# lambdaclass/ethrex

Hardware: NVIDIA H100
Metric: bn254_g1_msm_points_per_sec (higher is better)
Workload: dtype u32x8 Montgomery (254-bit modular integer)

## Files before the change

### ethrex_b200/csrc/msm.cu

```cuda
#include "common.cuh"
#include "tma.cuh"
#include <cstdlib>

namespace b200zk {

static constexpr int kMaxWindows = 64;
static constexpr uint32_t kMaxPipelineChunks = 64;
static constexpr int kChunk = 16;
static constexpr int kG2MinBlocks = 1;

struct MsmPlan {
  uint32_t c, W, B;
  uint32_t chunk, T;
  uint32_t merged;
  uint32_t Wr;
  uint32_t table_stride;
  uint32_t adaptive;
};

uint32_t precompute_window(size_t n) {
  uint32_t lg = 0;
  while (((size_t)1 << lg) < n) ++lg;
  if (lg >= 20) return 20;
  if (lg <= 6) return 6;
// ... 85 lines not shown

static constexpr uint32_t kHistTile = 256;
__global__ void __launch_bounds__(kHistTile) msm_hist(const void* scalars, size_t n, uint32_t flags, MsmPlan pl, uint32_t* hist, uint32_t* digits) {
  __shared__ __align__(128) uint4 tile[2][kHistTile * 2];
  __shared__ uint64_t bar[2];
  const size_t tiles = (n + kHistTile - 1) / kHistTile;
  if (threadIdx.x == 0) { tma::barrier_init(&bar[0], 1); tma::barrier_init(&bar[1], 1); tma::barrier_init_fence(); }
  __syncthreads();
  auto issue = [&](size_t tl, uint32_t buf) {
    size_t first = tl * kHistTile;
    uint32_t bytes = (uint32_t)((n - first < kHistTile ? n - first : kHistTile) * 32);
    tma::barrier_expect(&bar[buf], bytes);
    tma::bulk_load(tile[buf], reinterpret_cast<const uint8_t*>(scalars) + first * 32, bytes, &bar[buf]);
  };
  if (threadIdx.x == 0 && blockIdx.x < tiles) issue(blockIdx.x, 0);
  uint32_t it = 0;
  for (size_t tl = blockIdx.x; tl < tiles; tl += gridDim.x, ++it) {
    const uint32_t buf = it & 1;
    if (threadIdx.x == 0 && tl + gridDim.x < tiles) issue(tl + gridDim.x, buf ^ 1);
    tma::barrier_wait(&bar[buf], (it >> 1) & 1);
    const size_t i = tl * kHistTile + threadIdx.x;
    const bool live = i < n;
    uint32_t s[8] = {0, 0, 0, 0, 0, 0, 0, 0};
    if (live) decode_scalar(tile[buf][2 * threadIdx.x], tile[buf][2 * threadIdx.x + 1], flags, s);
    uint32_t carry = 0;
    for (uint32_t w = 0; w < pl.W; ++w) {
      uint32_t coef = window_bits(s, w, pl.c) + carry;
      carry = 0;
      uint32_t neg = 0, mag = coef;
      if (w + 1 < pl.W && coef >= pl.B) { carry = 1; neg = 0x80000000u; mag = (1u << pl.c) - coef; }
      uint32_t code = mag ? ((mag - 1) | neg) : kNoDigit;
      if (live) digits[(size_t)w * n + i] = code;
      uint32_t rank, gm;
      uint32_t cnt = warp_group(mag - 1, live && mag != 0, &rank, &gm, pl.adaptive != 0);
      if (live && mag && rank == 0) atomicAdd(&hist[(pl.merged ? 0 : (size_t)w * pl.B) + (mag - 1)], cnt);
    }
    __syncthreads();
  }
}

static constexpr int kScatterIlp = 4;
__global__ void __launch_bounds__(256) msm_scatter(const uint32_t* __restrict__ digits, size_t n, MsmPlan pl, uint32_t* cursor, uint32_t* idx) {
  const size_t total = (size_t)pl.W * n;
  const size_t stride = (size_t)gridDim.x * blockDim.x;
  const size_t total_pad = (total + 31) & ~(size_t)31;
  for (size_t t0 = blockIdx.x * (size_t)blockDim.x + threadIdx.x; t0 < total_pad; t0 += stride * kScatterIlp) {
    uint32_t code[kScatterIlp], g[kScatterIlp], rank[kScatterIlp], mask[kScatterIlp], base[kScatterIlp];
    size_t w[kScatterIlp];
    bool live[kScatterIlp], active[kScatterIlp];
#pragma unroll
    for (int u = 0; u < kScatterIlp; ++u) {
      const size_t t = t0 + u * stride;
      live[u] = t < total_pad;
      code[u] = (live[u] && t < total) ? __ldg(digits + t) : kNoDigit;
      active[u] = code[u] != kNoDigit;
      w[u] = live[u] ? t / n : 0;
      g[u] = (pl.merged ? 0u : (uint32_t)(w[u] * pl.B)) + (code[u] & 0x7fffffffu);
    }
#pragma unroll
    for (int u = 0; u < kScatterIlp; ++u) {
      base[u] = 0; rank[u] = 0; mask[u] = 0;
      if (live[u]) {
        uint32_t cnt = warp_group(g[u], active[u], &rank[u], &mask[u], pl.adaptive != 0);
        if (active[u] && rank[u] == 0) base[u] = atomicAdd(&cursor[g[u]], cnt);
      }
    }
#pragma unroll
    for (int u = 0; u < kScatterIlp; ++u) {
      if (live[u]) {
        uint32_t bs = __shfl_sync(mask[u], base[u], __ffs(mask[u]) - 1);
        const size_t t = t0 + u * stride;
        if (active[u]) idx[bs + rank[u]] = (uint32_t)((t - w[u] * n) + (pl.merged ? w[u] * pl.table_stride : 0)) | (code[u] & 0x80000000u);
      }
    }
  }
}

static constexpr uint32_t kSortTile = 1024;
static constexpr uint32_t kSortMaxW = 16;
static constexpr uint32_t kSortMaxBins = 1024;
static constexpr uint32_t kSortMaxFine = 2048;
static constexpr uint32_t kSortCountSub = 4;
static constexpr int kFineIlp = 8;

struct SortPlan {
  uint32_t fb;
  uint32_t C;
  uint32_t NC;
  uint32_t range;
  uint32_t G;
};
static bool make_sort_plan(size_t n, const MsmPlan& pl, int sm_count, SortPlan* sp) {
  const size_t G = (size_t)pl.Wr * pl.B;
  uint32_t kb = 0;
  while (((size_t)1 << kb) < G) ++kb;
  if (pl.W > kSortMaxW || kb < 12 || n < ((size_t)1 << 16)) return false;
  uint32_t cb = kb > 19 ? 10 : 9;
  if (kb - cb > 11) return false;
  sp->fb = kb - cb;
  sp->C = (uint32_t)((G + ((size_t)1 << sp->fb) - 1) >> sp->fb);
  sp->G = (uint32_t)G;
  uint32_t nc = (uint32_t)sm_count;
  size_t tiles = (n + kSortTile - 1) / kSortTile;
  if (nc > tiles) nc = (uint32_t)tiles;
  size_t per = ((tiles + nc - 1) / nc) * kSortTile;
  sp->NC = (uint32_t)((n + per - 1) / per);
  sp->range = (uint32_t)per;
  return true;
}

B2_D void recode_scalar(const uint32_t s[8], const MsmPlan& pl, uint32_t (&code)[kSortMaxW]) {
  uint32_t carry = 0;
#pragma unroll
  for (uint32_t w = 0; w < kSortMaxW; ++w) {
    code[w] = kNoDigit;
    if (w < pl.W) {
      uint32_t coef = window_bits(s, w, pl.c) + carry;
      carry = 0;
      uint32_t neg = 0, mag = coef;
      if (w + 1 < pl.W && coef >= pl.B) { carry = 1; neg = 0x80000000u; mag = (1u << pl.c) - coef; }
      code[w] = mag ? ((mag - 1) | neg) : kNoDigit;
    }
  }
}

__global__ void __launch_bounds__(kHistTile) msm_sort_count(const void* scalars, size_t n, uint32_t flags, MsmPlan pl, SortPlan sp, uint32_t* cnt) {
  __shared__ __align__(128) uint4 tile[2][kHistTile * 2];
  __shared__ uint64_t bar[2];
  __shared__ uint32_t sh[kSortMaxBins];
  const uint32_t r = blockIdx.x / kSortCountSub, sub = blockIdx.x % kSortCountSub;
  for (uint32_t b = threadIdx.x; b < sp.C; b += kHistTile) sh[b] = 0;
  const size_t lo = (size_t)r * sp.range, hi = lo + sp.range < n ? lo + sp.range : n;
  const size_t tiles_all = lo < hi ? (hi - lo + kHistTile - 1) / kHistTile : 0;
  const size_t per = (tiles_all + kSortCountSub - 1) / kSortCountSub;
  const size_t t0 = sub * per, t1 = t0 + per < tiles_all ? t0 + per : tiles_all;
  if (threadIdx.x == 0) { tma::barrier_init(&bar[0], 1); tma::barrier_init(&bar[1], 1); tma::barrier_init_fence(); }
  __syncthreads();
  auto issue = [&](size_t tl, uint32_t buf) {
    size_t first = lo + tl * kHistTile;
    uint32_t bytes = (uint32_t)((hi - first < kHistTile ? hi - first : kHistTile) * 32);
    tma::barrier_expect(&bar[buf], bytes);
    tma::bulk_load(tile[buf], reinterpret_cast<const uint8_t*>(scalars) + first * 32, bytes, &bar[buf]);
  };
  if (threadIdx.x == 0 && t0 < t1) issue(t0, 0);
  uint32_t it = 0;
  for (size_t tl = t0; tl < t1; ++tl, ++it) {
    const uint32_t buf = it & 1;
    if (threadIdx.x == 0 && tl + 1 < t1) issue(tl + 1, buf ^ 1);
    tma::barrier_wait(&bar[buf], (it >> 1) & 1);
    const size_t i = lo + tl * kHistTile + threadIdx.x;
    if (i < hi) {
      uint32_t s[8], code[kSortMaxW];
      decode_scalar(tile[buf][2 * threadIdx.x], tile[buf][2 * threadIdx.x + 1], flags, s);
      recode_scalar(s, pl, code);
#pragma unroll
      for (uint32_t w = 0; w < kSortMaxW; ++w)
        if (code[w] != kNoDigit) {
          const uint32_t g = (pl.merged ? 0u : w * pl.B) + (code[w] & 0x7fffffffu);
          atomicAdd(&sh[g >> sp.fb], 1u);
        }
    }
    __syncthreads();
  }
  __syncthreads();
  for (uint32_t b = threadIdx.x; b < sp.C; b += kHistTile) if (sh[b]) atomicAdd(&cnt[(size_t)b * sp.NC + r], sh[b]);
}

struct SortCoarseSmem {
  uint2 ent[kSortTile * kSortMaxW];
  uint32_t dst[kSortTile * kSortMaxW];
  uint32_t run_base[kSortMaxBins], tile_cnt[kSortMaxBins], tile_start[kSortMaxBins];
  uint32_t warp_tot[kSortTile / 32];
  uint32_t total;
};
__global__ void __launch_bounds__(kSortTile, 1) msm_sort_coarse(const void* __restrict__ scalars, size_t n, uint32_t flags, MsmPlan pl, SortPlan sp, const uint32_t* __restrict__ base,
                                                               uint2* __restrict__ ent1) {
  extern __shared__ __align__(16) uint8_t smem_raw[];
  SortCoarseSmem& sm = *reinterpret_cast<SortCoarseSmem*>(smem_raw);
  const uint32_t r = blockIdx.x, tid = threadIdx.x;
  const size_t lo = (size_t)r * sp.range, hi = lo + sp.range < n ? lo + sp.range : n;
  const uint32_t fmask = (1u << sp.fb) - 1u;
  for (uint32_t b = tid; b < sp.C; b += kSortTile) { sm.run_base[b] = __ldg(base + (size_t)b * sp.NC + r); sm.tile_cnt[b] = 0; }
  __syncthreads();
  const uint4* sc = reinterpret_cast<const uint4*>(scalars);
  for (size_t t0 = lo; t0 < hi; t0 += kSortTile) {
    const size_t i = t0 + tid;
    uint32_t code[kSortMaxW], rank[kSortMaxW];
    const bool live = i < hi;
#pragma unroll
    for (uint32_t w = 0; w < kSortMaxW; ++w) { code[w] = kNoDigit; rank[w] = 0; }
    if (live) {
      uint32_t s[8];
      decode_scalar(__ldg(sc + 2 * i), __ldg(sc + 2 * i + 1), flags, s);
      recode_scalar(s, pl, code);
#pragma unroll
      for (uint32_t w = 0; w < kSortMaxW; ++w)
        if (code[w] != kNoDigit) {
          const uint32_t g = (pl.merged ? 0u : w * pl.B) + (code[w] & 0x7fffffffu);
          rank[w] = atomicAdd(&sm.tile_cnt[g >> sp.fb], 1u);
        }
    }
    __syncthreads();
    {
      const uint32_t v = tid < sp.C ? sm.tile_cnt[tid] : 0;
      uint32_t incl = v;
#pragma unroll
      for (int o = 1; o < 32; o <<= 1) { uint32_t t = __shfl_up_sync(0xffffffffu, incl, o); if ((tid & 31) >= (unsigned)o) incl += t; }
      if ((tid & 31) == 31) sm.warp_tot[tid >> 5] = incl;
      __syncthreads();
      uint32_t wb = 0;
      for (uint32_t k = 0; k < (tid >> 5); ++k) wb += sm.warp_tot[k];
      if (tid < sp.C) sm.tile_start[tid] = wb + incl - v;
      if (tid == kSortTile - 1) sm.total = wb + incl;
    }
    __syncthreads();
    if (live) {
#pragma unroll
      for (uint32_t w = 0; w < kSortMaxW; ++w)
        if (code[w] != kNoDigit) {
          const uint32_t g = (pl.merged ? 0u : w * pl.B) + (code[w] & 0x7fffffffu);
          const uint32_t b = g >> sp.fb, pos = sm.tile_start[b] + rank[w];
          sm.ent[pos] = make_uint2((uint32_t)(i + (pl.merged ? (size_t)w * pl.table_stride : 0)) | (code[w] & 0x80000000u), g & fmask);
          sm.dst[pos] = sm.run_base[b] + rank[w];
        }
    }
    __syncthreads();
    const uint32_t total = sm.total;
    for (uint32_t t = tid; t < total; t += kSortTile) ent1[sm.dst[t]] = sm.ent[t];
    __syncthreads();
    if (tid < sp.C) { sm.run_base[tid] += sm.tile_cnt[tid]; sm.tile_cnt[tid] = 0; }
    __syncthreads();
  }
}

static constexpr uint32_t kFineTile = 8192;
static constexpr uint32_t kFineSeg = 4 * kFineTile;
struct SortFineSmem {
  uint32_t val[kFineTile], dst[kFineTile];
  uint32_t cur[kSortMaxFine], tcnt[kSortMaxFine], tstart[kSortMaxFine];
  uint32_t warp_tot[32];
  uint32_t total;
};
B2_D void scan_fine_keys(const uint32_t* in, uint32_t* out, uint32_t F, uint32_t* warp_tot, uint32_t* total) {
  const uint32_t tid = threadIdx.x, k0 = 2 * tid, k1 = 2 * tid + 1;
  const uint32_t v0 = k0 < F ? in[k0] : 0, v1 = k1 < F ? in[k1] : 0;
  uint32_t incl = v0 + v1;
#pragma unroll
  for (int o = 1; o < 32; o <<= 1) { uint32_t t = __shfl_up_sync(0xffffffffu, incl, o); if ((tid & 31) >= (unsigned)o) incl += t; }
  if ((tid & 31) == 31) warp_tot[tid >> 5] = incl;
  __syncthreads();
  uint32_t wb = 0;
  for (uint32_t k = 0; k < (tid >> 5); ++k) wb += warp_tot[k];
  const uint32_t ex = wb + incl - v0 - v1;
  if (k0 < F) out[k0] = ex;
  if (k1 < F) out[k1] = ex + v0;
  if (tid == 1023) *total = wb + incl;
  __syncthreads();
}
__global__ void __launch_bounds__(1024) msm_sort_items(const uint32_t* __restrict__ base, SortPlan sp, uint32_t* __restrict__ item_start) {
  __shared__ uint32_t wt[32];
  const uint32_t tid = threadIdx.x;
  uint32_t v = 0;
  if (tid < sp.C) { const uint32_t sz = __ldg(base + (size_t)(tid + 1) * sp.NC) - __ldg(base + (size_t)tid * sp.NC); v = (sz + kFineSeg - 1) / kFineSeg; }
  uint32_t incl = v;
#pragma unroll
  for (int o = 1; o < 32; o <<= 1) { uint32_t t = __shfl_up_sync(0xffffffffu, incl, o); if ((tid & 31) >= (unsigned)o) incl += t; }
  if ((tid & 31) == 31) wt[tid >> 5] = incl;
  __syncthreads();
  uint32_t wb = 0;
  for (uint32_t k = 0; k < (tid >> 5); ++k) wb += wt[k];
  if (tid < sp.C) item_start[tid] = wb + incl - v;
  if (tid == sp.C - 1) item_start[sp.C] = wb + incl;
}
B2_D uint32_t item_bin(const uint32_t* __restrict__ item_start, uint32_t C, uint32_t i) {
  uint32_t lo = 0, hi = C;
  while (hi - lo > 1) { uint32_t mid = (lo + hi) >> 1; if (__ldg(item_start + mid) <= i) lo = mid; else hi = mid; }
  return lo;
}
__global__ void __launch_bounds__(1024, 2) msm_sort_fine_count(const uint2* __restrict__ ent1, SortPlan sp, const uint32_t* __restrict__ base, const uint32_t* __restrict__ item_start,
                                                               uint32_t* __restrict__ cnt2) {
  __shared__ uint32_t fh[kSortMaxFine];
  const uint32_t i = blockIdx.x, tid = threadIdx.x, F = 1u << sp.fb;
  if (i >= __ldg(item_start + sp.C)) return;
  const uint32_t b = item_bin(item_start, sp.C, i);
  const uint32_t bs = __ldg(base + (size_t)b * sp.NC), be = __ldg(base + (size_t)(b + 1) * sp.NC);
  const uint32_t s0 = bs + (i - __ldg(item_start + b)) * kFineSeg, s1 = (be - s0 > kFineSeg) ? s0 + kFineSeg : be;
  for (uint32_t k = tid; k < F; k += 1024) fh[k] = 0;
  __syncthreads();
  for (uint32_t e0 = s0 + tid; e0 < s1; e0 += 1024 * kFineIlp) {
    uint32_t kk[kFineIlp];
#pragma unroll
    for (int u = 0; u < kFineIlp; ++u) { const uint32_t e = e0 + u * 1024; kk[u] = e < s1 ? __ldg(&ent1[e].y) : 0xffffffffu; }
#pragma unroll
    for (int u = 0; u < kFineIlp; ++u) if (kk[u] != 0xffffffffu) atomicAdd(&fh[kk[u]], 1u);
  }
  __syncthreads();
  for (uint32_t k = tid; k < F; k += 1024) cnt2[(size_t)i * F + k] = fh[k];
}
__global__ void __launch_bounds__(256) msm_sort_fine_prefix(SortPlan sp, const uint32_t* __restrict__ item_start, uint32_t* __restrict__ cnt2, uint32_t* __restrict__ hist) {
  const uint32_t F = 1u << sp.fb;
  const size_t t = blockIdx.x * (size_t)blockDim.x + threadIdx.x;
  if (t >= (size_t)sp.C * F) return;
  const uint32_t b = (uint32_t)(t >> sp.fb), k = (uint32_t)t & (F - 1);
  const uint32_t i0 = __ldg(item_start + b), i1 = __ldg(item_start + b + 1);
  uint32_t run = 0;
  for (uint32_t i = i0; i < i1; ++i) {
    const size_t at = (size_t)i * F + k;
    const uint32_t c = cnt2[at];
    cnt2[at] = run;
    run += c;
  }
  if (t < sp.G) hist[t] = run;
}
__global__ void __launch_bounds__(1024, 1) msm_sort_fine_place(const uint2* __restrict__ ent1, SortPlan sp, const uint32_t* __restrict__ base, const uint32_t* __restrict__ item_start,
                                                               const uint32_t* __restrict__ cnt2, const uint32_t* __restrict__ offsets, uint32_t* __restrict__ idx) {
  extern __shared__ __align__(16) uint8_t smem_raw[];
  SortFineSmem& sm = *reinterpret_cast<SortFineSmem*>(smem_raw);
  const uint32_t i = blockIdx.x, tid = threadIdx.x, F = 1u << sp.fb;
  if (i >= __ldg(item_start + sp.C)) return;
  const uint32_t b = item_bin(item_start, sp.C, i);
  const uint32_t bs = __ldg(base + (size_t)b * sp.NC), be = __ldg(base + (size_t)(b + 1) * sp.NC);
  const uint32_t s0 = bs + (i - __ldg(item_start + b)) * kFineSeg, s1 = (be - s0 > kFineSeg) ? s0 + kFineSeg : be;
  for (uint32_t k = tid; k < F; k += 1024) {
    const size_t g = (size_t)b * F + k;
    sm.cur[k] = (g < sp.G ? __ldg(offsets + g) : 0u) + __ldg(cnt2 + (size_t)i * F + k);
    sm.tcnt[k] = 0;
  }
  __syncthreads();
  for (uint32_t t0 = s0; t0 < s1; t0 += kFineTile) {
    uint2 ev[kFineTile / 1024];
    uint32_t rank[kFineTile / 1024];
#pragma unroll
    for (int u = 0; u < (int)(kFineTile / 1024); ++u) {
      const uint32_t e = t0 + u * 1024 + tid;
      ev[u] = e < s1 ? __ldg(ent1 + e) : make_uint2(0u, 0xffffffffu);
    }
#pragma unroll
    for (int u = 0; u < (int)(kFineTile / 1024); ++u) rank[u] = ev[u].y != 0xffffffffu ? atomicAdd(&sm.tcnt[ev[u].y], 1u) : 0u;
    __syncthreads();
    scan_fine_keys(sm.tcnt, sm.tstart, F, sm.warp_tot, &sm.total);
#pragma unroll
    for (int u = 0; u < (int)(kFineTile / 1024); ++u)
      if (ev[u].y != 0xffffffffu) {
        const uint32_t pos = sm.tstart[ev[u].y] + rank[u];
        sm.val[pos] = ev[u].x;
        sm.dst[pos] = sm.cur[ev[u].y] + rank[u];
      }
    __syncthreads();
    const uint32_t total = sm.total;
    for (uint32_t t = tid; t < total; t += 1024) idx[sm.dst[t]] = sm.val[t];
    __syncthreads();
    for (uint32_t k = tid; k < F; k += 1024) { sm.cur[k] += sm.tcnt[k]; sm.tcnt[k] = 0; }
    __syncthreads();
  }
}

static constexpr int kScanThreads = 256, kScanItems = 8, kScanTile = kScanThreads * kScanItems;

B2_D uint32_t scan_value(const uint32_t* in, const uint32_t* aux, size_t i, uint32_t seg, uint32_t shift) {
  uint32_t v = in[i];
  if (!seg) return (v + (1u << shift) - 1u) >> shift;
  return (v != 0 && (aux[i] % seg) != 0) ? 1u : 0u;
}

__global__ void __launch_bounds__(kScanThreads) scan_tile_sums(const uint32_t* in, const uint32_t* aux, size_t G, uint32_t seg, uint32_t shift, uint32_t* tile_sums) {
  __shared__ uint32_t red[kScanThreads / 32];
  size_t base = (size_t)blockIdx.x * kScanTile + (size_t)threadIdx.x * kScanItems;
  uint32_t s = 0;
#pragma unroll
  for (int k = 0; k < kScanItems; ++k) if (base + k < G) s += scan_value(in, aux, base + k, seg, shift);
#pragma unroll
  for (int o = 16; o; o >>= 1) s += __shfl_xor_sync(0xffffffffu, s, o);
  if ((threadIdx.x & 31) == 0) red[threadIdx.x >> 5] = s;
  __syncthreads();
  if (threadIdx.x == 0) {
    uint32_t t = 0;
    for (int k = 0; k < kScanThreads / 32; ++k) t += red[k];
    tile_sums[blockIdx.x] = t;
  }
}
__global__ void __launch_bounds__(1024) scan_tile_offsets(uint32_t* tile_sums, size_t tiles) {
  __shared__ uint32_t buf[1024];
  __shared__ uint32_t carry;
  if (threadIdx.x == 0) carry = 0;
  __syncthreads();
  for (size_t base = 0; base < tiles; base += 1024) {
    size_t i = base + threadIdx.x;
    uint32_t v = i < tiles ? tile_sums[i] : 0;
    buf[threadIdx.x] = v;
    __syncthreads();
    for (int o = 1; o < 1024; o <<= 1) {
      uint32_t t = threadIdx.x >= (unsigned)o ? buf[threadIdx.x - o] : 0;
      __syncthreads();
      buf[threadIdx.x] += t;
      __syncthreads();
    }
    uint32_t incl = buf[threadIdx.x], c0 = carry;
    __syncthreads();
    if (i < tiles) tile_sums[i] = c0 + incl - v;
    if (threadIdx.x == 1023) carry = c0 + incl;
    __syncthreads();
  }
}
__global__ void __launch_bounds__(kScanThreads) scan_apply(const uint32_t* in, const uint32_t* aux, size_t G, uint32_t seg, uint32_t shift, const uint32_t* tile_offsets, uint32_t* offsets, uint32_t* cursor) {
  __shared__ uint32_t warp_tot[kScanThreads / 32];
  size_t base = (size_t)blockIdx.x * kScanTile + (size_t)threadIdx.x * kScanItems;
  uint32_t v[kScanItems], s = 0;
#pragma unroll
  for (int k = 0; k < kScanItems; ++k) { v[k] = base + k < G ? scan_value(in, aux, base + k, seg, shift) : 0; s += v[k]; }
  uint32_t incl = s;
#pragma unroll
  for (int o = 1; o < 32; o <<= 1) { uint32_t t = __shfl_up_sync(0xffffffffu, incl, o); if ((threadIdx.x & 31) >= (unsigned)o) incl += t; }
  if ((threadIdx.x & 31) == 31) warp_tot[threadIdx.x >> 5] = incl;
  __syncthreads();
  uint32_t wbase = 0;
  for (unsigned k = 0; k < (threadIdx.x >> 5); ++k) wbase += warp_tot[k];
  uint32_t run = tile_offsets[blockIdx.x] + wbase + incl - s;
#pragma unroll
  for (int k = 0; k < kScanItems; ++k) {
    if (base + k < G) { offsets[base + k] = seg ? run + (aux[base + k] + seg - 1) / seg : run; if (cursor) cursor[base + k] = run; }
    run += v[k];
  }
  if (blockIdx.x == gridDim.x - 1 && threadIdx.x == kScanThreads - 1) offsets[G] = seg ? run + (aux[G] + seg - 1) / seg : run;
}

static constexpr uint32_t kSegLenMax = 256;
static constexpr uint32_t kTreeRadix = 64;
static constexpr uint32_t kDirectRuns = 4;

static uint32_t pick_slice_len(size_t M, size_t resident) {
  if (M == 0) return kSegLenMax;
  size_t per_thread = (M + resident - 1) / resident;
  size_t waves = (per_thread + kSegLenMax - 1) / kSegLenMax;
  size_t len = (M + resident * waves - 1) / (resident * waves);
  if (len < 16) len = 16;
  if (len > kSegLenMax) len = kSegLenMax;
  return (uint32_t)len;
// ... 480 lines not shown
  for (size_t k = 0; k < count; ++k) { XYZZ<F> p = load_xyzz<F>(partials, k); xyzz_add(acc, p); }
  Affine<F> a = xyzz_to_affine(acc);
  encode_point(out, a, native);
  *reinterpret_cast<uint32_t*>(out + 2 * FieldBytes<F>::value) = a.is_inf() ? 1u : 0u;
}

__global__ void groth16_assemble(const uint8_t* __restrict__ partials, size_t count, uint8_t* __restrict__ out) {
  if (threadIdx.x) return;
  const uint32_t which = blockIdx.x;
  uint32_t* inf = reinterpret_cast<uint32_t*>(out + 320);
  if (which == 1) {
    XYZZ<Fq2> acc = XYZZ<Fq2>::identity();
    for (size_t k = 0; k < count; ++k) { XYZZ<Fq2> p = load_xyzz<Fq2>(partials + k * 768 + 256, 0); xyzz_add(acc, p); }
    Affine<Fq2> a = xyzz_to_affine(acc);
    encode_point(out + 64, a, false);
    inf[1] = a.is_inf() ? 1u : 0u;
    return;
  }
  XYZZ<Fq> acc = XYZZ<Fq>::identity();
  const size_t off = which == 0 ? 0 : (which == 3 ? 128 : 512);
  for (size_t k = 0; k < count; ++k) {
    XYZZ<Fq> p = load_xyzz<Fq>(partials + k * 768 + off, 0);
    xyzz_add(acc, p);
    if (which == 2) { XYZZ<Fq> h = load_xyzz<Fq>(partials + k * 768 + 640, 0); xyzz_add(acc, h); }
  }
  Affine<Fq> a = xyzz_to_affine(acc);
  encode_point(out + (which == 0 ? 0 : (which == 2 ? 192 : 256)), a, false);
  inf[which == 0 ? 0 : (which == 2 ? 2 : 3)] = a.is_inf() ? 1u : 0u;
}
int groth16_assemble_dev(b200zk_ctx* ctx, const void* d_partials, size_t count, cudaStream_t st, void* d_out) {
  B2_LAUNCH(ctx, groth16_assemble, 4, 32, 0, st, (const uint8_t*)d_partials, count, (uint8_t*)d_out);
  return B200ZK_OK;
}

static inline void phase_mark(b200zk_ctx* ctx, int k, cudaStream_t st) {
  if (ctx->profiling) cudaEventRecord(ctx->ev[k], st);
}

static int g2_pair_knob() {
  static int k = -1;
  if (k < 0) { const char* e = getenv("B200ZK_G2_PAIR"); k = (e && (*e == '0' || *e == '3' || *e == '4')) ? (*e - '0') : 3; }
  return k;
}
template <class F> static size_t resident_slices(const b200zk_ctx* ctx) {
  if (IsFq2<F>::value) { const int k = g2_pair_knob(); return (size_t)ctx->sm_count * (k ? 64u * (unsigned)k : 256u); }
  return (size_t)ctx->sm_count * (sizeof(F) > 32 ? 256u : 512u);
}
template <class F>
static int launch_accumulate(b200zk_ctx* ctx, cudaStream_t st, const void* pts, const uint32_t* idx, const uint32_t* offsets, const uint32_t* run_off, uint32_t G, uint32_t L,
                             size_t slices, void* partials, uint32_t* run_bucket) {
  const unsigned agrid = (unsigned)((slices + 127) / 128);
  if constexpr (IsFq2<F>::value) {
    const int k = g2_pair_knob();
    const unsigned pgrid = (unsigned)((2 * slices + 127) / 128);
    if (k == 3) B2_LAUNCH(ctx, msm_accumulate_g2_pair<3>, pgrid, 128, 0, st, pts, idx, offsets, run_off, G, L, partials, run_bucket);
    else if (k == 4) B2_LAUNCH(ctx, msm_accumulate_g2_pair<4>, pgrid, 128, 0, st, pts, idx, offsets, run_off, G, L, partials, run_bucket);
    else B2_LAUNCH(ctx, (msm_accumulate<F, false, 1>), agrid, 128, 0, st, pts, idx, offsets, run_off, G, L, partials, run_bucket);
  } else {
    B2_LAUNCH(ctx, (msm_accumulate<F, false>), agrid, 128, 0, st, pts, idx, offsets, run_off, G, L, partials, run_bucket);
  }
  return B200ZK_OK;
}

static int legacy_sort_knob() {
  static int knob = -1;
  if (knob < 0) { const char* e = getenv("B200ZK_SORT"); knob = (e && !strcmp(e, "legacy")) ? 1 : 0; }
  return knob;
}
static double chunk_ratio_knob(double dflt) {
  const char* e = getenv("B200ZK_CHUNK_RATIO");
  double r = (e && *e) ? atof(e) : dflt;
  return (r >= 1.0 && r <= 64.0) ? r : dflt;
}
static size_t sort_ctab_bytes(int sm_count) { return (2 * ((size_t)kSortMaxBins * (size_t)sm_count + 1) + kSortMaxBins + 1) * 4; }
static size_t sort_cnt2_bytes(size_t M_max) { return (M_max / kFineSeg + kSortMaxBins + 1) * (size_t)kSortMaxFine * 4; }
static int run_two_level_sort(b200zk_ctx* ctx, const void* d_scalars, size_t n, uint32_t flags, const MsmPlan& pl, const SortPlan& sp, uint32_t* hist, uint32_t* offsets,
                              uint32_t* tsum, uint2* ent1, uint32_t* ctab, uint32_t* cnt2, uint32_t* idx, cudaStream_t st, bool mark) {
  const size_t Gc = (size_t)sp.C * sp.NC, tilesC = (Gc + kScanTile - 1) / kScanTile;
  const size_t G = sp.G, tilesG = (G + kScanTile - 1) / kScanTile;
  uint32_t *cnt = ctab, *base = ctab + Gc + 1, *item_start = base + Gc + 1;
  if (!ctx->attr_sort) {
    B2_CUDA(ctx, cudaFuncSetAttribute(msm_sort_coarse, cudaFuncAttributeMaxDynamicSharedMemorySize, (int)sizeof(SortCoarseSmem)));
    B2_CUDA(ctx, cudaFuncSetAttribute(msm_sort_fine_place, cudaFuncAttributeMaxDynamicSharedMemorySize, (int)sizeof(SortFineSmem)));
    ctx->attr_sort = true;
  }
  B2_CUDA(ctx, cudaMemsetAsync(cnt, 0, (Gc + 1) * 4, st));
  B2_LAUNCH(ctx, msm_sort_count, sp.NC * kSortCountSub, kHistTile, 0, st, d_scalars, n, flags, pl, sp, cnt);
  if (mark) phase_mark(ctx, 1, st);
  B2_LAUNCH(ctx, scan_tile_sums, (unsigned)tilesC, kScanThreads, 0, st, (const uint32_t*)cnt, (const uint32_t*)nullptr, Gc, 0u, 0u, tsum);
  B2_LAUNCH(ctx, scan_tile_offsets, 1, 1024, 0, st, tsum, tilesC);
  B2_LAUNCH(ctx, scan_apply, (unsigned)tilesC, kScanThreads, 0, st, (const uint32_t*)cnt, (const uint32_t*)nullptr, Gc, 0u, 0u, (const uint32_t*)tsum, base, (uint32_t*)nullptr);
  if (mark) phase_mark(ctx, 2, st);
  B2_LAUNCH(ctx, msm_sort_coarse, sp.NC, kSortTile, sizeof(SortCoarseSmem), st, d_scalars, n, flags, pl, sp, (const uint32_t*)base, ent1);
  const unsigned max_items = (unsigned)((n * (size_t)pl.W) / kFineSeg + sp.C + 1);
  const uint32_t F = 1u << sp.fb;
  B2_LAUNCH(ctx, msm_sort_items, 1, 1024, 0, st, (const uint32_t*)base, sp, item_start);
  B2_LAUNCH(ctx, msm_sort_fine_count, max_items, 1024, 0, st, (const uint2*)ent1, sp, (const uint32_t*)base, (const uint32_t*)item_start, cnt2);
  B2_LAUNCH(ctx, msm_sort_fine_prefix, (unsigned)(((size_t)sp.C * F + 255) / 256), 256, 0, st, sp, (const uint32_t*)item_start, cnt2, hist);
  B2_LAUNCH(ctx, scan_tile_sums, (unsigned)tilesG, kScanThreads, 0, st, (const uint32_t*)hist, (const uint32_t*)nullptr, G, 0u, 0u, tsum);
  B2_LAUNCH(ctx, scan_tile_offsets, 1, 1024, 0, st, tsum, tilesG);
  B2_LAUNCH(ctx, scan_apply, (unsigned)tilesG, kScanThreads, 0, st, (const uint32_t*)hist, (const uint32_t*)nullptr, G, 0u, 0u, (const uint32_t*)tsum, offsets, (uint32_t*)nullptr);
  B2_LAUNCH(ctx, msm_sort_fine_place, max_items, 1024, sizeof(SortFineSmem), st, (const uint2*)ent1, sp, (const uint32_t*)base, (const uint32_t*)item_start, (const uint32_t*)cnt2,
            (const uint32_t*)offsets, idx);
  return B200ZK_OK;
}

template <class F>
static int msm_run_pipelined(b200zk_ctx* ctx, const void* d_points, const void* d_scalars, const void* h_scalars, size_t n, uint32_t flags,
                             cudaStream_t st, void* d_partial, const MsmPlan& pl, uint32_t K) {
  const size_t G = (size_t)pl.Wr * pl.B;
  const size_t tiles = (G + kScanTile - 1) / kScanTile;
  const size_t xy = 4 * FieldBytes<F>::value, pt = 2 * FieldBytes<F>::value;
  size_t bnd[kMaxPipelineChunks + 1];
  uint32_t chunks = 0;
  {
    const double r = h_scalars ? chunk_ratio_knob(IsFq2<F>::value ? 12.0 : 4.0) : 1.0;
    double tot = 0, w = 1;
    for (uint32_t k = 0; k < K; ++k) { tot += w; w *= r; }
    double cum = 0; w = 1;
    bnd[0] = 0;
    for (uint32_t k = 0; k < K; ++k) {
      cum += w; w *= r;
      size_t hi = (k == K - 1) ? n : std::min(n, (((size_t)((double)n * (cum / tot))) + 1023) & ~(size_t)1023);
      if (hi > bnd[chunks]) bnd[++chunks] = hi;
    }
  }
  size_t chunk = 0;
  for (uint32_t k = 0; k < chunks; ++k) chunk = std::max(chunk, bnd[k + 1] - bnd[k]);
  const size_t Mk_max = chunk * pl.W;
  const size_t resident = resident_slices<F>(ctx);
  uint32_t Lk[kMaxPipelineChunks];
  size_t S_max = 0;
  for (uint32_t k = 0; k < chunks; ++k) {
    const size_t Mk = (bnd[k + 1] - bnd[k]) * pl.W;
    Lk[k] = pick_slice_len(Mk, resident);
    S_max = std::max(S_max, Mk / Lk[k] + 1 + G);
  }
  SortPlan sp0;
  const bool two_level = !legacy_sort_knob() && make_sort_plan(chunk, pl, ctx->sm_count, &sp0);
  const size_t Gc = (size_t)kSortMaxBins * (size_t)ctx->sm_count;
  for (int sl = 0; sl < 2; ++sl) {
    SortSlot& s = ctx->slot[sl];
    B2_TRY(ensure(ctx, s.hist, G * 4)); B2_TRY(ensure(ctx, s.offsets, (G + 1) * 4)); B2_TRY(ensure(ctx, s.cursor, G * 4));
    B2_TRY(ensure(ctx, s.run_off, (G + 1) * 4));
    B2_TRY(ensure(ctx, s.tsum, std::max(tiles, (Gc + kScanTile - 1) / kScanTile) * 4));
    B2_TRY(ensure(ctx, s.digits, Mk_max * 4)); B2_TRY(ensure(ctx, s.idx, Mk_max * 4));
    if (two_level) { B2_TRY(ensure(ctx, s.key, Mk_max * 8)); B2_TRY(ensure(ctx, s.ctab, sort_ctab_bytes(ctx->sm_count))); B2_TRY(ensure(ctx, s.cnt2, sort_cnt2_bytes(Mk_max))); }
  }
  B2_TRY(ensure(ctx, ctx->ws_buckets, S_max * xy));
  B2_TRY(ensure(ctx, ctx->ws_segbucket, S_max * 4));
  B2_TRY(ensure(ctx, ctx->ws_totals, G * xy));
  B2_TRY(ensure(ctx, ctx->ws_chunkS, (size_t)pl.Wr * pl.T * xy));
  B2_TRY(ensure(ctx, ctx->ws_chunkV, (size_t)pl.Wr * pl.T * xy));
  if (h_scalars) B2_TRY(ensure(ctx, ctx->ws_scalars, n * 32 + 32));
  const uint8_t* dsc = (const uint8_t*)(h_scalars ? ctx->ws_scalars.p : d_scalars);
  cudaStream_t cs = ctx->stream_sort;
  if (h_scalars) {
    B2_CUDA(ctx, cudaEventRecord(ctx->ev_in, st));
    B2_CUDA(ctx, cudaStreamWaitEvent(cs, ctx->ev_in, 0));
    if (chunks > kMaxPipelineChunks) return fail(ctx, B200ZK_ERR_INVALID_ARG, "msm: too many pipeline chunks");
    for (uint32_t k = 0; k < chunks; ++k) {
      const size_t lo = bnd[k], nk = bnd[k + 1] - lo;
      B2_CUDA(ctx, cudaMemcpyAsync((void*)(dsc + lo * 32), (const uint8_t*)h_scalars + lo * 32, nk * 32, cudaMemcpyHostToDevice, cs));
      B2_CUDA(ctx, cudaEventRecord(ctx->ev_up[k], cs));
    }
  }
  auto sort_chunk = [&](uint32_t k) -> int {
    const size_t lo = bnd[k], nk = bnd[k + 1] - lo;
    const uint32_t L = Lk[k];
    SortSlot& s = ctx->slot[k & 1];
    uint32_t *hist = (uint32_t*)s.hist.p, *offsets = (uint32_t*)s.offsets.p, *cursor = (uint32_t*)s.cursor.p, *run_off = (uint32_t*)s.run_off.p,
             *tsum = (uint32_t*)s.tsum.p, *digits = (uint32_t*)s.digits.p, *idx = (uint32_t*)s.idx.p;
    if (h_scalars) B2_CUDA(ctx, cudaStreamWaitEvent(st, ctx->ev_up[k], 0));
    SortPlan sp;
    const bool tl = two_level && make_sort_plan(nk, pl, ctx->sm_count, &sp);
    if (tl) {
      B2_TRY(run_two_level_sort(ctx, (const void*)(dsc + lo * 32), nk, flags, pl, sp, hist, offsets, tsum, (uint2*)s.key.p, (uint32_t*)s.ctab.p, (uint32_t*)s.cnt2.p, idx, st, false));
    } else {
      B2_CUDA(ctx, cudaMemsetAsync(hist, 0, G * 4, st));
      const unsigned sgrid = (unsigned)std::min<size_t>((nk + 255) / 256, (size_t)ctx->sm_count * 8);
      B2_LAUNCH(ctx, msm_hist, sgrid, 256, 0, st, (const void*)(dsc + lo * 32), nk, flags, pl, hist, digits);
      B2_LAUNCH(ctx, scan_tile_sums, (unsigned)tiles, kScanThreads, 0, st, hist, (const uint32_t*)nullptr, G, 0u, 0u, tsum);
      B2_LAUNCH(ctx, scan_tile_offsets, 1, 1024, 0, st, tsum, tiles);
      B2_LAUNCH(ctx, scan_apply, (unsigned)tiles, kScanThreads, 0, st, hist, (const uint32_t*)nullptr, G, 0u, 0u, tsum, offsets, cursor);
      const unsigned wgrid = (unsigned)std::min<size_t>((nk * (size_t)pl.W + 255) / 256, (size_t)ctx->sm_count * 32);
      B2_LAUNCH(ctx, msm_scatter, wgrid, 256, 0, st, (const uint32_t*)digits, nk, pl, cursor, idx);
// ... 242 lines not shown
```

Baseline: 350.3 million.

## Restructure MSM two-level sort with TMA-staged scalars and single-pass fine placement

After: 362.2 million, median of 6. +3.4%, better.

```diff
diff --git a/ethrex_b200/csrc/msm.cu b/ethrex_b200/csrc/msm.cu
--- a/ethrex_b200/csrc/msm.cu
+++ b/ethrex_b200/csrc/msm.cu
@@ -191,6 +191,7 @@
 static constexpr uint32_t kSortMaxFine = 2048;
 static constexpr uint32_t kSortCountSub = 4;
 static constexpr int kFineIlp = 8;
+static constexpr uint16_t kNoFine = 0xffffu;
 
 struct SortPlan {
   uint32_t fb;
@@ -219,16 +220,27 @@
 }
 
 B2_D void recode_scalar(const uint32_t s[8], const MsmPlan& pl, uint32_t (&code)[kSortMaxW]) {
-  uint32_t carry = 0;
+  uint32_t t[9];
+#pragma unroll
+  for (int k = 0; k < 8; ++k) t[k] = s[k];
+  t[8] = 0;
+  const uint32_t mask = (1u << pl.c) - 1u;
+  uint32_t carry = 0, off = 0;
 #pragma unroll
   for (uint32_t w = 0; w < kSortMaxW; ++w) {
     code[w] = kNoDigit;
     if (w < pl.W) {
-      uint32_t coef = window_bits(s, w, pl.c) + carry;
+      uint32_t coef = (__funnelshift_r(t[0], t[1], off) & mask) + carry;
       carry = 0;
       uint32_t neg = 0, mag = coef;
       if (w + 1 < pl.W && coef >= pl.B) { carry = 1; neg = 0x80000000u; mag = (1u << pl.c) - coef; }
       code[w] = mag ? ((mag - 1) | neg) : kNoDigit;
+      off += pl.c;
+      if (off >= 32) {
+        off -= 32;
+#pragma unroll
+        for (int k = 0; k < 8; ++k) t[k] = t[k + 1];
+      }
     }
   }
 }
@@ -275,24 +287,55 @@
   for (uint32_t b = threadIdx.x; b < sp.C; b += kHistTile) if (sh[b]) atomicAdd(&cnt[(size_t)b * sp.NC + r], sh[b]);
 }
 
+template <uint32_t kThreads, uint32_t kMax>
+B2_D void scan_block(const uint32_t* in, uint32_t* out, uint32_t count, uint32_t* warp_tot, uint32_t* total) {
+  constexpr uint32_t kPer = kMax / kThreads;
+  const uint32_t tid = threadIdx.x;
+  uint32_t v[kPer], sum = 0;
+#pragma unroll
+  for (uint32_t j = 0; j < kPer; ++j) { const uint32_t k = tid * kPer + j; v[j] = k < count ? in[k] : 0; sum += v[j]; }
+  uint32_t incl = sum;
+#pragma unroll
+  for (int o = 1; o < 32; o <<= 1) { uint32_t t = __shfl_up_sync(0xffffffffu, incl, o); if ((tid & 31) >= (unsigned)o) incl += t; }
+  if ((tid & 31) == 31) warp_tot[tid >> 5] = incl;
+  __syncthreads();
+  uint32_t ex = incl - sum;
+  for (uint32_t k = 0; k < (tid >> 5); ++k) ex += warp_tot[k];
+  if (tid == kThreads - 1) *total = ex + sum;
+#pragma unroll
+  for (uint32_t j = 0; j < kPer; ++j) { const uint32_t k = tid * kPer + j; if (k < count) out[k] = ex; ex += v[j]; }
+  __syncthreads();
+}
+
 struct SortCoarseSmem {
+  uint4 sc[2][kSortTile * 2];
   uint2 ent[kSortTile * kSortMaxW];
-  uint32_t dst[kSortTile * kSortMaxW];
   uint32_t run_base[kSortMaxBins], tile_cnt[kSortMaxBins], tile_start[kSortMaxBins];
+  uint64_t bar[2];
   uint32_t warp_tot[kSortTile / 32];
   uint32_t total;
 };
 __global__ void __launch_bounds__(kSortTile, 1) msm_sort_coarse(const void* __restrict__ scalars, size_t n, uint32_t flags, MsmPlan pl, SortPlan sp, const uint32_t* __restrict__ base,
                                                                uint2* __restrict__ ent1) {
-  extern __shared__ __align__(16) uint8_t smem_raw[];
+  extern __shared__ __align__(128) uint8_t smem_raw[];
   SortCoarseSmem& sm = *reinterpret_cast<SortCoarseSmem*>(smem_raw);
   const uint32_t r = blockIdx.x, tid = threadIdx.x;
   const size_t lo = (size_t)r * sp.range, hi = lo + sp.range < n ? lo + sp.range : n;
   const uint32_t fmask = (1u << sp.fb) - 1u;
   for (uint32_t b = tid; b < sp.C; b += kSortTile) { sm.run_base[b] = __ldg(base + (size_t)b * sp.NC + r); sm.tile_cnt[b] = 0; }
-  __syncthreads();
-  const uint4* sc = reinterpret_cast<const uint4*>(scalars);
-  for (size_t t0 = lo; t0 < hi; t0 += kSortTile) {
+  if (tid == 0) { tma::barrier_init(&sm.bar[0], 1); tma::barrier_init(&sm.bar[1], 1); tma::barrier_init_fence(); }
+  __syncthreads();
+  auto issue = [&](size_t first, uint32_t buf) {
+    const uint32_t bytes = (uint32_t)((hi - first < kSortTile ? hi - first : kSortTile) * 32);
+    tma::barrier_expect(&sm.bar[buf], bytes);
+    tma::bulk_load(sm.sc[buf], reinterpret_cast<const uint8_t*>(scalars) + first * 32, bytes, &sm.bar[buf]);
+  };
+  if (tid == 0 && lo < hi) issue(lo, 0);
+  uint32_t it = 0;
+  for (size_t t0 = lo; t0 < hi; t0 += kSortTile, ++it) {
+    const uint32_t buf = it & 1;
+    if (tid == 0 && t0 + kSortTile < hi) issue(t0 + kSortTile, buf ^ 1);
+    tma::barrier_wait(&sm.bar[buf], (it >> 1) & 1);
     const size_t i = t0 + tid;
     uint32_t code[kSortMaxW], rank[kSortMaxW];
     const bool live = i < hi;
@@ -300,7 +343,7 @@
     for (uint32_t w = 0; w < kSortMaxW; ++w) { code[w] = kNoDigit; rank[w] = 0; }
     if (live) {
       uint32_t s[8];
-      decode_scalar(__ldg(sc + 2 * i), __ldg(sc + 2 * i + 1), flags, s);
+      decode_scalar(sm.sc[buf][2 * tid], sm.sc[buf][2 * tid + 1], flags, s);
       recode_scalar(s, pl, code);
 #pragma unroll
       for (uint32_t w = 0; w < kSortMaxW; ++w)
@@ -310,62 +353,40 @@
         }
     }
     __syncthreads();
-    {
-      const uint32_t v = tid < sp.C ? sm.tile_cnt[tid] : 0;
-      uint32_t incl = v;
-#pragma unroll
-      for (int o = 1; o < 32; o <<= 1) { uint32_t t = __shfl_up_sync(0xffffffffu, incl, o); if ((tid & 31) >= (unsigned)o) incl += t; }
-      if ((tid & 31) == 31) sm.warp_tot[tid >> 5] = incl;
-      __syncthreads();
-      uint32_t wb = 0;
-      for (uint32_t k = 0; k < (tid >> 5); ++k) wb += sm.warp_tot[k];
-      if (tid < sp.C) sm.tile_start[tid] = wb + incl - v;
-      if (tid == kSortTile - 1) sm.total = wb + incl;
-    }
-    __syncthreads();
+    scan_block<kSortTile, kSortMaxBins>(sm.tile_cnt, sm.tile_start, sp.C, sm.warp_tot, &sm.total);
     if (live) {
 #pragma unroll
       for (uint32_t w = 0; w < kSortMaxW; ++w)
         if (code[w] != kNoDigit) {
           const uint32_t g = (pl.merged ? 0u : w * pl.B) + (code[w] & 0x7fffffffu);
-          const uint32_t b = g >> sp.fb, pos = sm.tile_start[b] + rank[w];
-          sm.ent[pos] = make_uint2((uint32_t)(i + (pl.merged ? (size_t)w * pl.table_stride : 0)) | (code[w] & 0x80000000u), g & fmask);
-          sm.dst[pos] = sm.run_base[b] + rank[w];
+          const uint32_t pos = sm.tile_start[g >> sp.fb] + rank[w];
+          sm.ent[pos] = make_uint2((uint32_t)(i + (pl.merged ? (size_t)w * pl.table_stride : 0)) | (code[w] & 0x80000000u), g);
         }
     }
     __syncthreads();
     const uint32_t total = sm.total;
-    for (uint32_t t = tid; t < total; t += kSortTile) ent1[sm.dst[t]] = sm.ent[t];
+    for (uint32_t t = tid; t < total; t += kSortTile) {
+      const uint2 e = sm.ent[t];
+      const uint32_t b = e.y >> sp.fb;
+      ent1[sm.run_base[b] + (t - sm.tile_start[b])] = make_uint2(e.x, e.y & fmask);
+    }
     __syncthreads();
-    if (tid < sp.C) { sm.run_base[tid] += sm.tile_cnt[tid]; sm.tile_cnt[tid] = 0; }
+    for (uint32_t b = tid; b < sp.C; b += kSortTile) { sm.run_base[b] += sm.tile_cnt[b]; sm.tile_cnt[b] = 0; }
     __syncthreads();
   }
 }
 
-static constexpr uint32_t kFineTile = 8192;
-static constexpr uint32_t kFineSeg = 4 * kFineTile;
+static constexpr uint32_t kFineSeg = 32768;
+static constexpr uint32_t kFineThreads = 1024;
 struct SortFineSmem {
-  uint32_t val[kFineTile], dst[kFineTile];
-  uint32_t cur[kSortMaxFine], tcnt[kSortMaxFine], tstart[kSortMaxFine];
-  uint32_t warp_tot[32];
+  uint32_t val[kFineSeg];
+  uint16_t key[kFineSeg];
+  uint32_t cnt[kSortMaxFine];
+  uint32_t slot[kSortMaxFine];
+  uint32_t shift[kSortMaxFine];
+  uint32_t warp_tot[kFineThreads / 32];
   uint32_t total;
 };
-B2_D void scan_fine_keys(const uint32_t* in, uint32_t* out, uint32_t F, uint32_t* warp_tot, uint32_t* total) {
-  const uint32_t tid = threadIdx.x, k0 = 2 * tid, k1 = 2 * tid + 1;
-  const uint32_t v0 = k0 < F ? in[k0] : 0, v1 = k1 < F ? in[k1] : 0;
-  uint32_t incl = v0 + v1;
-#pragma unroll
-  for (int o = 1; o < 32; o <<= 1) { uint32_t t = __shfl_up_sync(0xffffffffu, incl, o); if ((tid & 31) >= (unsigned)o) incl += t; }
-  if ((tid & 31) == 31) warp_tot[tid >> 5] = incl;
-  __syncthreads();
-  uint32_t wb = 0;
-  for (uint32_t k = 0; k < (tid >> 5); ++k) wb += warp_tot[k];
-  const uint32_t ex = wb + incl - v0 - v1;
-  if (k0 < F) out[k0] = ex;
-  if (k1 < F) out[k1] = ex + v0;
-  if (tid == 1023) *total = wb + incl;
-  __syncthreads();
-}
 __global__ void __launch_bounds__(1024) msm_sort_items(const uint32_t* __restrict__ base, SortPlan sp, uint32_t* __restrict__ item_start) {
   __shared__ uint32_t wt[32];
   const uint32_t tid = threadIdx.x;
@@ -399,9 +420,9 @@
   for (uint32_t e0 = s0 + tid; e0 < s1; e0 += 1024 * kFineIlp) {
     uint32_t kk[kFineIlp];
 #pragma unroll
-    for (int u = 0; u < kFineIlp; ++u) { const uint32_t e = e0 + u * 1024; kk[u] = e < s1 ? __ldg(&ent1[e].y) : 0xffffffffu; }
-#pragma unroll
-    for (int u = 0; u < kFineIlp; ++u) if (kk[u] != 0xffffffffu) atomicAdd(&fh[kk[u]], 1u);
+    for (int u = 0; u < kFineIlp; ++u) { const uint32_t e = e0 + u * 1024; kk[u] = e < s1 ? __ldg(&ent1[e].y) : kNoFine; }
+#pragma unroll
+    for (int u = 0; u < kFineIlp; ++u) if (kk[u] != kNoFine) atomicAdd(&fh[kk[u]], 1u);
   }
   __syncthreads();
   for (uint32_t k = tid; k < F; k += 1024) cnt2[(size_t)i * F + k] = fh[k];
@@ -421,8 +442,9 @@
   }
   if (t < sp.G) hist[t] = run;
 }
-__global__ void __launch_bounds__(1024, 1) msm_sort_fine_place(const uint2* __restrict__ ent1, SortPlan sp, const uint32_t* __restrict__ base, const uint32_t* __restrict__ item_start,
-                                                               const uint32_t* __restrict__ cnt2, const uint32_t* __restrict__ offsets, uint32_t* __restrict__ idx) {
+__global__ void __launch_bounds__(kFineThreads, 1) msm_sort_fine_place(const uint2* __restrict__ ent1, SortPlan sp, const uint32_t* __restrict__ base,
+                                                                       const uint32_t* __restrict__ item_start, const uint32_t* __restrict__ cnt2, const uint32_t* __restrict__ hist,
+                                                                       const uint32_t* __restrict__ offsets, uint32_t* __restrict__ idx) {
   extern __shared__ __align__(16) uint8_t smem_raw[];
   SortFineSmem& sm = *reinterpret_cast<SortFineSmem*>(smem_raw);
   const uint32_t i = blockIdx.x, tid = threadIdx.x, F = 1u << sp.fb;
@@ -430,38 +452,36 @@
   const uint32_t b = item_bin(item_start, sp.C, i);
   const uint32_t bs = __ldg(base + (size_t)b * sp.NC), be = __ldg(base + (size_t)(b + 1) * sp.NC);
   const uint32_t s0 = bs + (i - __ldg(item_start + b)) * kFineSeg, s1 = (be - s0 > kFineSeg) ? s0 + kFineSeg : be;
-  for (uint32_t k = tid; k < F; k += 1024) {
+  const bool last = __ldg(item_start + b + 1) == i + 1;
+  for (uint32_t k = tid; k < F; k += kFineThreads) {
     const size_t g = (size_t)b * F + k;
-    sm.cur[k] = (g < sp.G ? __ldg(offsets + g) : 0u) + __ldg(cnt2 + (size_t)i * F + k);
-    sm.tcnt[k] = 0;
-  }
-  __syncthreads();
-  for (uint32_t t0 = s0; t0 < s1; t0 += kFineTile) {
-    uint2 ev[kFineTile / 1024];
-    uint32_t rank[kFineTile / 1024];
-#pragma unroll
-    for (int u = 0; u < (int)(kFineTile / 1024); ++u) {
-      const uint32_t e = t0 + u * 1024 + tid;
-      ev[u] = e < s1 ? __ldg(ent1 + e) : make_uint2(0u, 0xffffffffu);
-    }
-#pragma unroll
-    for (int u = 0; u < (int)(kFineTile / 1024); ++u) rank[u] = ev[u].y != 0xffffffffu ? atomicAdd(&sm.tcnt[ev[u].y], 1u) : 0u;
-    __syncthreads();
-    scan_fine_keys(sm.tcnt, sm.tstart, F, sm.warp_tot, &sm.total);
-#pragma unroll
-    for (int u = 0; u < (int)(kFineTile / 1024); ++u)
-      if (ev[u].y != 0xffffffffu) {
-        const uint32_t pos = sm.tstart[ev[u].y] + rank[u];
-        sm.val[pos] = ev[u].x;
-        sm.dst[pos] = sm.cur[ev[u].y] + rank[u];
+    const uint32_t pre = __ldg(cnt2 + (size_t)i * F + k);
+    const uint32_t next = last ? (g < sp.G ? __ldg(hist + g) : 0u) : __ldg(cnt2 + (size_t)(i + 1) * F + k);
+    sm.cnt[k] = next - pre;
+    sm.shift[k] = (g < sp.G ? __ldg(offsets + g) : 0u) + pre;
+  }
+  __syncthreads();
+  scan_block<kFineThreads, kSortMaxFine>(sm.cnt, sm.slot, F, sm.warp_tot, &sm.total);
+  for (uint32_t k = tid; k < F; k += kFineThreads) sm.shift[k] -= sm.slot[k];
+  __syncthreads();
+  for (uint32_t e0 = s0 + tid; e0 < s1; e0 += kFineThreads * kFineIlp) {
+    uint2 ev[kFineIlp];
+#pragma unroll
+    for (int u = 0; u < kFineIlp; ++u) {
+      const uint32_t e = e0 + u * kFineThreads;
+      ev[u] = e < s1 ? __ldg(ent1 + e) : make_uint2(0u, kNoFine);
+    }
+#pragma unroll
+    for (int u = 0; u < kFineIlp; ++u)
+      if (ev[u].y != kNoFine) {
+        const uint32_t p = atomicAdd(&sm.slot[ev[u].y], 1u);
+        sm.val[p] = ev[u].x;
+        sm.key[p] = (uint16_t)ev[u].y;
       }
-    __syncthreads();
-    const uint32_t total = sm.total;
-    for (uint32_t t = tid; t < total; t += 1024) idx[sm.dst[t]] = sm.val[t];
-    __syncthreads();
-    for (uint32_t k = tid; k < F; k += 1024) { sm.cur[k] += sm.tcnt[k]; sm.tcnt[k] = 0; }
-    __syncthreads();
-  }
+  }
+  __syncthreads();
+  const uint32_t total = s1 - s0;
+  for (uint32_t t = tid; t < total; t += kFineThreads) idx[t + sm.shift[sm.key[t]]] = sm.val[t];
 }
 
 static constexpr int kScanThreads = 256, kScanItems = 8, kScanTile = kScanThreads * kScanItems;
@@ -1108,6 +1128,7 @@
   if (!ctx->attr_sort) {
     B2_CUDA(ctx, cudaFuncSetAttribute(msm_sort_coarse, cudaFuncAttributeMaxDynamicSharedMemorySize, (int)sizeof(SortCoarseSmem)));
     B2_CUDA(ctx, cudaFuncSetAttribute(msm_sort_fine_place, cudaFuncAttributeMaxDynamicSharedMemorySize, (int)sizeof(SortFineSmem)));
+    B2_CUDA(ctx, cudaFuncSetAttribute(msm_sort_fine_place, cudaFuncAttributePreferredSharedMemoryCarveout, (int)cudaSharedmemCarveoutMaxShared));
     ctx->attr_sort = true;
   }
   B2_CUDA(ctx, cudaMemsetAsync(cnt, 0, (Gc + 1) * 4, st));
@@ -1126,8 +1147,8 @@
   B2_LAUNCH(ctx, scan_tile_sums, (unsigned)tilesG, kScanThreads, 0, st, (const uint32_t*)hist, (const uint32_t*)nullptr, G, 0u, 0u, tsum);
   B2_LAUNCH(ctx, scan_tile_offsets, 1, 1024, 0, st, tsum, tilesG);
   B2_LAUNCH(ctx, scan_apply, (unsigned)tilesG, kScanThreads, 0, st, (const uint32_t*)hist, (const uint32_t*)nullptr, G, 0u, 0u, (const uint32_t*)tsum, offsets, (uint32_t*)nullptr);
-  B2_LAUNCH(ctx, msm_sort_fine_place, max_items, 1024, sizeof(SortFineSmem), st, (const uint2*)ent1, sp, (const uint32_t*)base, (const uint32_t*)item_start, (const uint32_t*)cnt2,
-            (const uint32_t*)offsets, idx);
+  B2_LAUNCH(ctx, msm_sort_fine_place, max_items, kFineThreads, sizeof(SortFineSmem), st, (const uint2*)ent1, sp, (const uint32_t*)base,
+            (const uint32_t*)item_start, (const uint32_t*)cnt2, (const uint32_t*)hist, (const uint32_t*)offsets, idx);
   return B200ZK_OK;
 }
 
```
